# google-deepmind/spriteworld

Measured on AMD Instinct MI355X. Metric: env-steps/sec (incl. 64x64 RGB render) at 8192 envs, higher is better.
Workload: dtype i32 fixed-point raster/resample + f64 state

## Files before the change

include/swb.h:

```cpp
#ifndef SWB_H_
#define SWB_H_

#include <stdint.h>

#ifdef __cplusplus
extern "C" {
#endif

#define SWB_MAX_SPRITES 64
#define SWB_MAX_TASKS 8
#define SWB_MAX_SHAPES 32
#define SWB_MAX_SHAPE_VERTS 64
#define SWB_MAX_CUTS 4
#define SWB_MAX_CELLS ((SWB_MAX_CUTS + 1) * (SWB_MAX_CUTS + 1))

enum swb_status {
  SWB_OK = 0,
  SWB_ERR_INVALID = -1,
  SWB_ERR_HIP = -2,
  SWB_ERR_NO_DEVICE = -3,
  SWB_ERR_STATE = -4
};

enum swb_action_space {
// ... 261 lines not shown

#define SWB_ALL_STEPS (-1)
int swb_rollout_step_frames(swb_handle h, int32_t M, int32_t step, const int32_t* cand_dev, uint8_t* obs_dev, uint8_t* error_dev,
                            void* stream);

#define SWB_CONTAINED_MAX_TRIES 1024
enum swb_action_sampling { SWB_SAMPLE_UNIFORM = 0, SWB_SAMPLE_ON_SPRITE = 1 };
typedef struct swb_sampled_actions {
  void* actions;
  double* position;
  int32_t* sprite;
  int32_t* tries;
} swb_sampled_actions;
int swb_sample_actions(swb_handle h, int32_t mode, uint64_t seed, uint64_t first_env, const swb_sampled_actions* out, void* stream);

typedef struct swb_rollout_sampled_outputs {
  void*    actions;
  int32_t* sprite;
  int32_t* tries;
} swb_rollout_sampled_outputs;
int swb_rollout_sampled(swb_handle h, int32_t mode , uint64_t seed, uint64_t first_env,
                        int32_t M, int32_t K, int32_t keep_steps, const swb_rollout_outputs* out,
                        const swb_rollout_step_outputs* steps, const swb_rollout_sampled_outputs* sampled, void* stream);

int swb_trim_run_lists(swb_handle h, int32_t* run_cap_out, void* stream);

int swb_list_stats(swb_handle h, int64_t* kept, int64_t* built, void* stream);

int swb_frame_stats(swb_handle h, int64_t* copied, int64_t* filled, int64_t* resampled, void* stream);
int swb_frame_cycles(swb_handle h, int64_t* out3, void* stream);

int swb_split_stats(swb_handle h, int64_t* whole, int64_t* bands, int64_t* whole_copies, void* stream);

int swb_factors(swb_handle h, double* factors_dev, void* stream);

int swb_get_env_state(swb_handle h, int32_t env, int32_t* out5, void* stream);
int swb_get_sprite_types(swb_handle h, int32_t env, int32_t sprite, int32_t* flags, void* stream);

int swb_get_state(swb_handle h, const swb_state* host_state, void* stream);
int swb_set_positions(swb_handle h, const double* x_host, const double* y_host, void* stream);

typedef struct swb_snapshot {
  double *x, *y;
  int32_t *n_sprites, *pool_entry, *step_count, *episode, *pool_base, *pool_len;
  uint8_t *reset_next;
} swb_snapshot;
enum swb_state_source { SWB_STATE_LIVE = 0, SWB_STATE_ROLLOUT_END = 1 };
int swb_pool_id(swb_handle h, uint64_t* id);
int swb_save_state(swb_handle h, int32_t source, const int32_t* index_dev, int32_t C, const swb_snapshot* snap, void* stream);
int swb_load_state(swb_handle h, const swb_snapshot* snap, int32_t C, const int32_t* slot_dev, uint64_t pool_id,
                   int32_t* rejected_dev, void* stream);

int swb_copy_pool(swb_handle dst, swb_handle src, const int32_t* pool_base_host, const int32_t* pool_len_host, void* stream);

enum swb_sprite_attr { SWB_ATTR_SHAPE = 0, SWB_ATTR_ANGLE = 1, SWB_ATTR_SCALE = 2 };
int swb_set_sprite_attr(swb_handle h, int32_t env, int32_t sprite, int32_t attr, double value, const double* delta,
                        const int8_t* label, void* stream);

int swb_set_sprite_cell_labels(swb_handle h, int32_t env, int32_t sprite, const int8_t* cells, void* stream);

int swb_get_sprite(swb_handle h, int32_t env, int32_t sprite, int32_t* shape, double* angle, double* scale, int32_t* n_verts,
                   double* path_xy, void* stream);

int swb_sprite_path_op(int32_t attr, double a, double b, int32_t n, const double* in_xy, double* out_xy);

typedef struct swb_variant_info {
  int32_t nw;
  int32_t ncol;
  int32_t vs;
  int32_t lds_bytes_per_wave;
  int32_t waves_per_simd;
  int32_t resample_waves_per_simd;
  int32_t n_bands;
  int32_t n_column_groups;
  int32_t run_cap;
  int32_t paint_in_cover;
  int32_t arena_units;
  int32_t large_frames;
  int32_t many_sprites;
  int32_t reserved_;
  int64_t run_list_bytes;
  int64_t frame_cache_bytes;
  int32_t split_bands;
  int32_t split_pad_;
} swb_variant_info;
int swb_variant(swb_handle h, swb_variant_info* out);
const char* swb_build_id(void);

int swb_timing_enable(swb_handle h, int32_t enable);
int swb_step_time_ms(swb_handle h, double* total_ms, int64_t* launches);
int swb_kernel_times_ms(swb_handle h, double* cover_ms, double* resample_ms, int64_t* launches);

#ifdef __cplusplus
}
#endif
#endif
```

spriteworld_amd/_abi.py:

```python
import ctypes as C

SWB_MAX_SPRITES = 64
SWB_TUNED_SPRITES = 16
SWB_MAX_TASKS = 8
SWB_MAX_SHAPES = 32
SWB_MAX_SHAPE_VERTS = 64
SWB_MAX_GROUPS = 8
SWB_MAX_CUTS = 4
SWB_MAX_CELLS = (SWB_MAX_CUTS + 1) * (SWB_MAX_CUTS + 1)
SWB_MAX_CANDIDATES = 12

ACTION_SELECT_MOVE, ACTION_DRAG_AND_DROP, ACTION_EMBODIED = 0, 1, 2
TASK_NO_REWARD, TASK_FIND_GOAL, TASK_CLUSTERING = 0, 1, 2
AGG_SUM, AGG_MAX, AGG_MIN, AGG_MEAN = 0, 1, 2, 3
TERM_ALL, TERM_ANY = 0, 1
STEP_FIRST, STEP_MID, STEP_LAST = 0, 1, 2
ENV_ERR_DB_ZERO, ENV_ERR_DB_LABELS, ENV_ERR_SPAN_OVERFLOW = 1, 2, 4
ATTR_SHAPE, ATTR_ANGLE, ATTR_SCALE = 0, 1, 2
SAMPLE_UNIFORM, SAMPLE_ON_SPRITE = 0, 1
SWB_CONTAINED_MAX_TRIES = 1024


class SwbTask(C.Structure):
  _fields_ = [
# ... 117 lines not shown
      ('x', C.c_void_p),
      ('y', C.c_void_p),
      ('n_sprites', C.c_void_p),
      ('pool_entry', C.c_void_p),
      ('step_count', C.c_void_p),
      ('reset_next', C.c_void_p),
      ('episode', C.c_void_p),
  ]


class SwbSnapshot(C.Structure):
  _fields_ = [
      ('x', C.c_void_p),
      ('y', C.c_void_p),
      ('n_sprites', C.c_void_p),
      ('pool_entry', C.c_void_p),
      ('step_count', C.c_void_p),
      ('episode', C.c_void_p),
      ('pool_base', C.c_void_p),
      ('pool_len', C.c_void_p),
      ('reset_next', C.c_void_p),
  ]


STATE_LIVE, STATE_ROLLOUT_END = 0, 1


class SwbVariantInfo(C.Structure):
  _fields_ = [('nw', C.c_int32), ('ncol', C.c_int32), ('vs', C.c_int32), ('lds_bytes_per_wave', C.c_int32),
              ('waves_per_simd', C.c_int32), ('resample_waves_per_simd', C.c_int32), ('n_bands', C.c_int32),
              ('n_column_groups', C.c_int32), ('run_cap', C.c_int32), ('paint_in_cover', C.c_int32),
              ('arena_units', C.c_int32), ('large_frames', C.c_int32), ('many_sprites', C.c_int32), ('reserved_', C.c_int32),
              ('run_list_bytes', C.c_int64), ('frame_cache_bytes', C.c_int64),
              ('split_bands', C.c_int32), ('split_pad_', C.c_int32)]


FACTOR_UNIFORM_F32, FACTOR_UNIFORM_INT, FACTOR_DISCRETE = 0, 1, 2


class SwbFactor(C.Structure):
  _fields_ = [
      ('kind', C.c_int32),
      ('n', C.c_int32),
      ('lo', C.c_double),
      ('hi', C.c_double),
      ('cand', C.c_double * SWB_MAX_CANDIDATES),
  ]


FACTOR_ORDER = ('x', 'y', 'scale', 'angle', 'c0', 'c1', 'c2', 'x_vel', 'y_vel')
SWB_N_FACTORS = len(FACTOR_ORDER)
SWB_MAX_HOLDOUTS = 2


class SwbHoldout(C.Structure):
  _fields_ = [
      ('redraw_mask', C.c_uint32),
      ('box_mask', C.c_uint32),
      ('lo', C.c_double * SWB_N_FACTORS),
      ('hi', C.c_double * SWB_N_FACTORS),
  ]


class SwbSpriteGroup(C.Structure):

  def factor(self, key):
    return self.factors[FACTOR_ORDER.index(key)]
# ... 203 lines not shown
```

spriteworld_amd/csrc/swb.hip:

```cpp
#include <hip/hip_runtime.h>

#include <algorithm>
#include <atomic>
#include <cmath>
#include <cstdarg>
#include <cstdio>
#include <cstdlib>
#include <cstring>
#include <memory>
#include <string>
#include <vector>

#include "swb_kernels.hip.inc"
#include "swb_pow.hip.inc"
#include "swb_sampler.hip.inc"

extern template __global__ void swb_cover_kernel<20, false>(const swb_params);
extern template __global__ void swb_cover_kernel<20, true>(const swb_params);

namespace {

thread_local std::string g_err;

int fail(int code, const char* fmt, ...) {
// ... 890 lines not shown
    if (per_xcd >= 2 && (per_xcd & (per_xcd - 1)) == 0 && rs_waves <= (long long)h->cus * 4 * SWB_RS_WAVES_PER_SIMD && !getenv("SWB_NO_SNAKE"))
      while ((1 << p.deal_shift) < per_xcd) ++p.deal_shift;
    if (const char* x = getenv("SWB_DEAL_SHIFT")) p.deal_shift = std::max(0, atoi(x));
  }
  h->run_cap_worst = std::max(4, p.S + 1) * p.Hc + 1;
  p.run_cap = h->run_cap_worst;
  if (const char* x = getenv("SWB_RUN_CAP")) p.run_cap = std::max(8, atoi(x));
  if (const char* x = getenv("SWB_ARENA_UNITS")) h->arena_override = std::max(0, atoi(x));
  const size_t NS = (size_t)p.N * p.S;
  if (h->d_x.fill(nullptr, NS) || h->d_y.fill(nullptr, NS) || h->d_nspr.fill(nullptr, p.N) || h->d_entry.fill(nullptr, p.N) ||
      h->d_step_count.fill(nullptr, p.N) || h->d_episode.fill(nullptr, p.N) || h->d_reset_next.fill(nullptr, p.N))
    return SWB_ERR_HIP;
  if (getenv("SWB_LIST_STATS")) {
    if (h->d_list_stats.fill(nullptr, 2) || h->d_frame_stats.fill(nullptr, 6)) return SWB_ERR_HIP;
    p.list_stats = h->d_list_stats;
    p.frame_stats = h->d_frame_stats;
    if (h->split_bands) {
      if (h->d_split_stats.fill(nullptr, 3)) return SWB_ERR_HIP;
      p.split_stats = h->d_split_stats;
    }
  }
  h->copy_cost = h->split_bands ? SWB_SPLIT_COPY_COST : SWB_COPY_COST;
  if (const char* x = getenv("SWB_COPY_COST")) h->copy_cost = std::max(0, atoi(x));
  if (p.AA != 1 && !h->large_frames && !h->no_keep_lists && !getenv("SWB_NO_FRAME_CACHE")) {
    const size_t bytes = (size_t)p.N * p.Wo * p.Ho * 3;
    if (hipMalloc(reinterpret_cast<void**>(&h->d_frame_cache.ptr), bytes) == hipSuccess) {
      h->d_frame_cache.count = bytes;
      p.frame_cache = h->d_frame_cache;
    } else {
      h->d_frame_cache.ptr = nullptr;
      (void)hipGetLastError();
    }
  }
  p.max_spans = SWB_MIN_SPANS;
  if (const char* ms = getenv("SWB_MAX_SPANS")) p.max_spans = atoi(ms) < SWB_MIN_SPANS ? SWB_MIN_SPANS : atoi(ms);
  p.span_cap = p.max_spans;
  if (const char* sc = getenv("SWB_LDS_SPAN_CAP")) p.span_cap = std::max(0, std::min(atoi(sc), p.max_spans));
  p.ovf_cap = std::min(p.Wc / 2 + 1, 32);
  p.ovf = nullptr;
  p.x = h->d_x; p.y = h->d_y; p.nspr = h->d_nspr; p.entry = h->d_entry; p.step_count = h->d_step_count;
  p.episode = h->d_episode; p.reset_next = h->d_reset_next;
  *out = owner.release();
  return SWB_OK;
}

int swb_destroy(swb_handle h) {
  if (!h) return SWB_OK;
  (void)hipSetDevice(h->device);
  for (auto* list : {&h->events, &h->event_pool})
    for (auto& ev : *list) { (void)hipEventDestroy(ev.e0); (void)hipEventDestroy(ev.e1); (void)hipEventDestroy(ev.e2); }
  delete h;
  return SWB_OK;
}

int swb_upload_shapes(swb_handle h, const double* verts, const int32_t* offsets, int32_t n_shapes) {
  if (!h || !verts || !offsets) return fail(SWB_ERR_INVALID, "null argument");
  bump_list_epoch(h);
  if (n_shapes < 1 || n_shapes > SWB_MAX_SHAPES) return fail(SWB_ERR_INVALID, "n_shapes must be in [1, %d]", SWB_MAX_SHAPES);
  HIP_TRY(hipSetDevice(h->device));
  int maxv = 0;
  for (int i = 0; i < n_shapes; ++i) {
    const int n = offsets[i + 1] - offsets[i];
    if (n < 3 || n > SWB_MAX_SHAPE_VERTS) return fail(SWB_ERR_INVALID, "shape %d has %d vertices (3..%d supported)", i, n, SWB_MAX_SHAPE_VERTS);
    if (n > maxv) maxv = n;
  }
  std::vector<double> dmin(n_shapes, 0.0);
// ... 1149 lines not shown
  if (shape) *shape = r.shape[sprite];
  if (angle) *angle = r.angle[sprite];
  if (scale) *scale = r.scale[sprite];
  if (n_verts) *n_verts = nv;
  if (path_xy) memcpy(path_xy, r.cpath.data() + (size_t)sprite * SWB_MAX_SHAPE_VERTS * 2, (size_t)nv * 16);
  return SWB_OK;
}

int swb_variant(swb_handle h, swb_variant_info* out) {
  if (!h || !out) return fail(SWB_ERR_INVALID, "null argument");
  if (h->large_frames) {
    const variant* v0 = &kVariants[0];
    out->nw = v0->nw; out->ncol = 1; out->vs = 0;
    out->lds_bytes_per_wave = (int32_t)lds_per_wave(h, v0, nullptr);
    out->waves_per_simd = SWB_COVER_WAVES(v0->nw);
    out->resample_waves_per_simd = 0;
    out->n_bands = 0;
    out->n_column_groups = 0;
    out->run_cap = 0;
    out->paint_in_cover = 0;
    out->arena_units = 0;
    out->large_frames = 1;
    out->many_sprites = h->many_sprites ? 1 : 0;
    out->reserved_ = 0;
    if (h->many_sprites) {
      out->nw = 0;
      out->lds_bytes_per_wave = (int32_t)sizeof(swb_ms_lds);
      out->waves_per_simd = 0;
    }
    out->run_list_bytes = 0;
    out->frame_cache_bytes = 0;
    out->split_bands = 0;
    out->split_pad_ = 0;
    return SWB_OK;
  }
  const variant* v = pick_variant(h->p.Wc);
  if (!v) return fail(SWB_ERR_INVALID, "canvas %dx%d not supported", h->p.Wc, h->p.Hc);
  int vs = 0;
  (void)pick_resample(h->p.AA, h->vslots, &vs);
  out->nw = v->nw; out->ncol = 1; out->vs = vs;
  out->lds_bytes_per_wave = (int32_t)lds_per_wave(h, v, nullptr);
  out->waves_per_simd = SWB_COVER_WAVES(v->nw);
  out->resample_waves_per_simd = SWB_RS_WAVES_PER_SIMD;
  out->n_bands = h->split_bands ? 1 : (h->p.nbands ? h->p.nbands : h->nbands);
  out->split_bands = h->split_bands ? (h->p.nbands ? h->p.nbands : h->nbands) : 0;
  out->split_pad_ = 0;
  out->n_column_groups = h->p.ncg;
  out->run_cap = h->p.run_cap;
  out->paint_in_cover = paints_in_cover(h, v) ? 1 : 0;
  out->arena_units = h->d_runs ? h->p.arena_units : 0;
  out->large_frames = 0;
  out->many_sprites = 0;
  out->reserved_ = 0;
  out->run_list_bytes = h->d_runs ? ((int64_t)h->p.arena_base + h->p.arena_units + 4) * 8 : 0;
  out->frame_cache_bytes = (int64_t)h->d_frame_cache.count;
  return SWB_OK;
}

#ifndef SWB_BUILD_ID
#define SWB_BUILD_ID "unknown"
#endif
const char* swb_build_id(void) { return SWB_BUILD_ID; }

int swb_timing_enable(swb_handle h, int32_t enable) {
  if (!h) return fail(SWB_ERR_INVALID, "null handle");
  HIP_TRY(hipSetDevice(h->device));
  if (flush_timing(h)) return SWB_ERR_HIP;
  h->timing = enable != 0;
  h->timed_ms = 0.0;
  h->timed_cover_ms = 0.0;
  h->timed_launches = 0;
  return SWB_OK;
}

int swb_step_time_ms(swb_handle h, double* total_ms, int64_t* launches) {
  if (!h) return fail(SWB_ERR_INVALID, "null handle");
  HIP_TRY(hipSetDevice(h->device));
  if (flush_timing(h)) return SWB_ERR_HIP;
  if (total_ms) *total_ms = h->timed_ms;
// ... 16 lines not shown
```

spriteworld_amd/csrc/swb_kernels.hip.inc:

```
#include <hip/hip_runtime.h>
#include <stdint.h>

#include "../../include/swb.h"

#define SWB_WAVE 64
#ifndef SWB_WORD_GROUPS
#define SWB_WORD_GROUPS 4
#endif
#ifndef SWB_AES_MIN_ITERS
#define SWB_AES_MIN_ITERS 4
#endif
#ifndef SWB_AES_MAX_NARROW_NW
#define SWB_AES_MAX_NARROW_NW 10
#endif
#ifndef SWB_COVER_WAVES_PER_SIMD
#define SWB_COVER_WAVES_PER_SIMD 5
#endif
#ifndef SWB_COVER_WAVES_PER_SIMD_NARROW
#define SWB_COVER_WAVES_PER_SIMD_NARROW 6
#endif
#ifndef SWB_COVER_WAVES_PER_SIMD_WIDE
#define SWB_COVER_WAVES_PER_SIMD_WIDE 4
#endif
#ifndef SWB_RS_WAVES_PER_SIMD
// ... 69 lines not shown
  const uint32_t* v_break;
  const int32_t* cg_lo;
  const int32_t* cg_hi;
  uint32_t* cost_cnt;
  int32_t* cost_list;
  int32_t cost_cap;
  int32_t cost_range0;
  int32_t parity;
  int32_t deal_shift;
  int32_t* ccost_list;
  int32_t cover_order;
  int32_t cphase;
  int32_t prio_div;
  int32_t prio_levels;
  int32_t paint_in_cover;
  int32_t band_tasks;
  uint8_t* ov_flag;
  const int32_t* ov_shape;
  const double* ov_scale;
  const double* ov_angle;
  const int8_t* ov_label;
  const double* ov_cpath;
  const int8_t* ov_cell_label;
  uint32_t list_epoch;
  uint32_t list_pad_;
  unsigned long long* list_stats;
  uint8_t* frame_cache;
  unsigned long long* frame_stats;
  int32_t obs_aligned16;
  int32_t copy_cost;
  int32_t split_bands;
  int32_t split_when;
  int32_t split_carry;
  int32_t split_pad_;
  unsigned long long* split_stats;
};

template <typename T>
using cptr = const T __attribute__((address_space(4)))*;
template <typename T>
__device__ __forceinline__ cptr<T> as_const(const T* q) { return (cptr<T>)(uintptr_t)q; }

__device__ __forceinline__ int lane_id() { return threadIdx.x & (SWB_WAVE - 1); }
__device__ __forceinline__ int rfl(int v) { return __builtin_amdgcn_readfirstlane(v); }
__device__ __forceinline__ float rflf(float v) { return __int_as_float(__builtin_amdgcn_readfirstlane(__float_as_int(v))); }
__device__ __forceinline__ double rfld(double v) {
  const long long b = __double_as_longlong(v);
  const int lo = __builtin_amdgcn_readfirstlane((int)(b & 0xffffffffll));
  const int hi = __builtin_amdgcn_readfirstlane((int)(b >> 32));
  return __longlong_as_double(((long long)hi << 32) | (unsigned int)lo);
}
__device__ __forceinline__ double readlane_d(double v, int src) {
  const long long b = __double_as_longlong(v);
  const int lo = __builtin_amdgcn_readlane((int)(b & 0xffffffffll), src);
  const int hi = __builtin_amdgcn_readlane((int)(b >> 32), src);
  return __longlong_as_double(((long long)hi << 32) | (unsigned int)lo);
}
__device__ __forceinline__ void wave_sync() {
  __builtin_amdgcn_fence(__ATOMIC_ACQ_REL, "wavefront");
  __builtin_amdgcn_wave_barrier();
}
__device__ __forceinline__ int wave_min_i(int v) {
  for (int o = 32; o > 0; o >>= 1) v = min(v, __shfl_xor(v, o, 64));
  return v;
}
__device__ __forceinline__ int wave_max_i(int v) {
  for (int o = 32; o > 0; o >>= 1) v = max(v, __shfl_xor(v, o, 64));
// ... 1364 lines not shown
        }                                                                                                         \
      } while (0)
      SWB_LIST_SPAN(rs.s0, 0 < cnt);
      SWB_LIST_SPAN(rs.s1, 1 < cnt);
      SWB_LIST_SPAN(rs.s2, 2 < cnt);
      for (int i = SWB_REG_SPANS; i < maxc; ++i) SWB_LIST_SPAN(lane_span(p, spans, ovf, rs, i, l), i < cnt);
#undef SWB_LIST_SPAN
      if (start && fc > SWB_REG_SPANS && ((fc - 3) & 1)) dst[2 * (2 + ((fc - 3) >> 1)) + 1] = 0u;
    }
    while (next_band_g < p.nbands) {
      const int y0 = as_const(p.band_y0)[next_band_g];
      if (y0 > yb + 63) break;
      const int at = base_g + ((y0 <= yb || !room) ? 0 : __builtin_amdgcn_readlane(excl, (y0 - yb) & 63));
      if (l == 0) hdr[SWB_RHDR_GROUPS + g * SWB_RHDR_GSTRIDE + 1 + next_band_g] = (uint32_t)at;
      if (bst && l == 0) bst[g * SWB_BST_STRIDE + next_band_g] = (uint32_t)at;
      ++next_band_g;
    }
    const int cost_g = SWB_RUN_COST * __popcll(__ballot(start)) + SWB_UNIT_COST * (total - __popcll(__ballot(contin)));
    if (l == g) { base_l = room ? base_g + total : base_g; band_l = (int)((meta_g & ~15u) | (uint32_t)next_band_g); cost_l += room ? cost_g : 0; }
  }
}

#define SWB_RESCAN_WITH_OVERFLOW_SLOT()                                                          \
  if (__ballot((err & SWB_INT_NEED_SLOT) != 0u)) {                                               \
    err &= ~SWB_INT_NEED_SLOT;                                                                   \
    if (rfl(*ovf) == -1) {                                                                       \
      if (l == 0) *ovf = ovf_slot_alloc(p);                                                      \
      wave_sync();                                                                               \
      if (rfl(*ovf) >= 0) { yb -= 64; continue; }                                                \
    }                                                                                            \
    err |= SWB_ENV_ERR_SPAN_OVERFLOW;                                                            \
  }

template <int NW, bool OV = false, bool PAINT = false>
__global__ void __launch_bounds__(SWB_WAVE, SWB_COVER_WAVES(NW))
swb_cover_kernel(const swb_params p) {
  static_assert(!PAINT || NW == 2, "painting in the cover kernel: images of up to 64 columns at anti_aliasing = 1");
  extern __shared__ __attribute__((aligned(16))) unsigned char smem[];
  const int l = lane_id();
  const uint32_t cycles0 = (uint32_t)__builtin_amdgcn_s_memtime();
  int env = blockIdx.x;
  uint32_t predicted = 0u, prio_q = 0u;
  int prio = 0;
  const int ph = p.cphase, ph_prev = ph == 0 ? 2 : ph - 1, ph_next = ph == 2 ? 0 : ph + 1;
  uint32_t filing_words_l = 0u;
  if (p.cost_cnt != nullptr && l < ((!PAINT && p.split_bands) ? 4 : 3))
    filing_words_l = p.cost_cnt[l == 0 ? SWB_COST_WORD_KEY_LO(p.parity) : (l == 1 ? SWB_COST_WORD_KEY_SCALE(p.parity) : ((PAINT || l == 2) ? SWB_COST_WORD_COVER_SHIFT(ph) : SWB_COST_WORD_SPLIT(p.parity)))];
  if (p.ccost_list) cover_cost_housekeeping(p, ph_prev, ph, ph_next);
  if (p.arena_head != nullptr && blockIdx.x == 0 && l == 0) p.arena_head[p.parity ^ 1] = 0u;
  if (p.cover_order) {
    const int sh = (int)(blockIdx.x & (SWB_COST_SHARDS - 1)), cap = (p.N + SWB_COST_SHARDS - 1) / SWB_COST_SHARDS;
    int bucket = 0;
    env = cost_ordered_entry(p.cost_cnt + cost_row1(ph_prev, sh),
                             as_const(p.ccost_list) + (size_t)(ph_prev * SWB_COST_SHARDS + sh) * SWB_COST_BUCKETS * cap, cap,
                             (int)(blockIdx.x >> 3), &bucket);
    if (env < 0) return;
    prio_q = (p.prio_levels & 2) ? as_const(p.cost_cnt)[SWB_COST_WORD_COVER_PRIO(ph)] : 0u;
    if (prio_q) predicted = (uint32_t)(2 * bucket + 1) << (as_const(p.cost_cnt)[SWB_COST_WORD_COVER_SHIFT(ph_prev)] - 1u);
  }
  auto file_cover_cost = [&]() __attribute__((always_inline)) {
    if (p.ccost_list) {
      const uint32_t cycles = (uint32_t)__builtin_amdgcn_s_memtime() - cycles0;
      const uint32_t width = (uint32_t)__builtin_amdgcn_readlane((int)filing_words_l, 2);
      if (l == 0) {
        const int key = (int)min(cycles >> width, (uint32_t)(SWB_COST_BUCKETS - 1));
        const int sh = env & (SWB_COST_SHARDS - 1);
// ... 59 lines not shown
    if (k < vtotal) {
      double cx, cy;
      bool from_table = true;
      if constexpr (OV) {
        if (es.ov) {
          const double* q = p.ov_cpath + (((size_t)env * S + sid) * SWB_MAX_SHAPE_VERTS + i) * 2;
          cx = q[0]; cy = q[1];
          from_table = false;
        }
      }
      if (from_table) centered_vertex(p, so, i, sc, ca, sa, cx, cy);
      cpath[k] = make_double2(cx, cy);
    }
  }
  wave_sync();
  SWB_HOOK_PHASE_END(3)

  auto hit = [&](int s2, double tx, double ty) __attribute__((always_inline)) {
    return contains_point_wave(cpath + __builtin_amdgcn_readlane(voff_l, s2), __builtin_amdgcn_readlane(nv_l, s2), tx, ty);
  };
  const step_cost sc = act_and_move(p, env, es, hit);
  const double px = es.px, py = es.py;
  SWB_HOOK_PHASE_END(4)
  if (p.render_only != 1) {
    err |= finish_step<OV>(p, env, es, sc, tscratch);
    wave_sync();
  }
  SWB_HOOK_PHASE_END(5)
  if (p.obs == nullptr) {
    if (l == 0 && p.error && err) p.error[env] |= (uint8_t)err;
    return;
  }

  [[maybe_unused]] auto file_lists = [&](int cost_l, const uint32_t* bst, uint32_t built_cycles, bool copies) __attribute__((always_inline)) {
    const bool whole = p.split_bands && (copies || __builtin_amdgcn_readlane((int)filing_words_l, 3) == 0);
    const bool bt = bst != nullptr && !whole;
    const int ntask = bt ? p.ncg * p.nbands : p.ncg;
    const bool file0 = p.cost_cnt != nullptr && l < ntask, file1 = p.ccost_list != nullptr && l == 0;
    const int sh = env & (SWB_COST_SHARDS - 1);
    int task_cost = cost_l, task_bits = l << 24;
    if (bt) {
      wave_sync();
      const int g2 = min(l / p.nbands, p.ncg - 1), b2 = l - (l / p.nbands) * p.nbands;
      const uint32_t* bg = bst + g2 * SWB_BST_STRIDE;
      const int u0 = (int)bg[b2], u1 = (int)bg[min(b2 + 1, p.nbands)], u2 = (int)bg[min(b2 + 2, p.nbands)];
      task_cost = 4 * max((u1 - u0) + (p.AA == 1 ? 0 : (((u2 - u1) * 5) >> 4)), 0);
      task_bits = (g2 << 24) | (b2 << 26);
    }
    if (whole) task_bits |= SWB_TASK_WHOLE;
    if (copies) task_cost = p.copy_cost;
    const int key0 = cost_key(task_cost, (uint32_t)__builtin_amdgcn_readlane((int)filing_words_l, 0), (uint32_t)__builtin_amdgcn_readlane((int)filing_words_l, 1));
    int key1 = 0;
    uint32_t cycles = built_cycles;
    if (p.ccost_list) {
      if (built_cycles == 0u) cycles = (uint32_t)__builtin_amdgcn_s_memtime() - cycles0;
      const uint32_t width = (uint32_t)__builtin_amdgcn_readlane((int)filing_words_l, 2);
      key1 = (int)min(cycles >> width, (uint32_t)(SWB_COST_BUCKETS - 1));
      if (l == 0 && (cycles >> width) >= (uint32_t)SWB_COST_BUCKETS) atomicMax(&p.cost_cnt[SWB_COST_WORD_COVER_MAX(ph, sh)], cycles);
    }
    uint32_t pos0 = 0u, pos1 = 0u;
    if (copies) { if (file0 && l == 0) pos0 = atomicAdd(&p.cost_cnt[cost_row0(p.parity, sh) + key0], (uint32_t)ntask); }
    else if (file0) pos0 = atomicAdd(&p.cost_cnt[cost_row0(p.parity, sh) + key0], 1u);
    if (file1) pos1 = atomicAdd(&p.cost_cnt[cost_row1(ph, sh) + key1], 1u);
    if (p.split_bands && !copies && p.cost_cnt != nullptr && l == 0) atomicAdd(&p.cost_cnt[SWB_COST_WORD_SPLIT_CNT(p.parity, sh, (env >> 3) & (SWB_COST_BUCKETS - 1))], (uint32_t)p.ncg);
    if (copies) pos0 = (uint32_t)__builtin_amdgcn_readlane((int)pos0, 0) + (uint32_t)l;
    if (file0) p.cost_list[((size_t)(p.parity * SWB_COST_SHARDS + sh) * SWB_COST_BUCKETS + key0) * p.cost_cap + pos0] = env | task_bits;
    if (file1) p.ccost_list[((size_t)(ph * SWB_COST_SHARDS + sh) * SWB_COST_BUCKETS + key1) * ((p.N + SWB_COST_SHARDS - 1) / SWB_COST_SHARDS) + pos1] = env;
    if (l == 0) ovf_slot_release(p, ovf);
    if (p.error) {
      uint32_t e = err & ~SWB_INT_NEED_SLOT;
      for (int o = 32; o > 0; o >>= 1) e |= (uint32_t)__shfl_xor((int)e, o, 64);
      if (l == 0 && e) p.error[env] |= (uint8_t)e;
    }
    return cycles;
  };

  if constexpr (!PAINT) {
    bool keep = false;
    uint32_t keep_words_l = 0u;
    if (p.list_epoch != 0u) {
      if (l <= SWB_MAX_CG + 2) keep_words_l = L->outrow[l];
      keep = (uint32_t)__builtin_amdgcn_readlane((int)keep_words_l, SWB_MAX_CG) == p.list_epoch && __ballot(es.first) == 0ull && !sc.changed;
    }
    if (p.list_stats != nullptr && l == 0) atomicAdd(&p.list_stats[keep ? 0 : 1], 1ull);
    if (keep) {
      const uint32_t frame_word_was = (uint32_t)__builtin_amdgcn_readlane((int)keep_words_l, SWB_MAX_CG + 2);
      const uint32_t frame_word = p.frame_cache ? min(frame_word_was + 1u, 2u) : 0u;
      uint32_t* bst = nullptr;
      const bool files_whole = p.split_bands && (frame_word == 2u || __builtin_amdgcn_readlane((int)filing_words_l, 3) == 0);
      if (p.band_tasks && !files_whole) {
        bst = L->outrow + 64;
        const uint32_t* hg = p.rhdr + (size_t)env * SWB_RHDR_DWORDS + SWB_RHDR_GROUPS;
        const int g = l / SWB_BST_STRIDE, b = l - g * SWB_BST_STRIDE;
        if (g < p.ncg && b <= p.nbands) bst[l] = hg[g * SWB_RHDR_GSTRIDE + (b < p.nbands ? 1 + b : 0)];
      }
      if (l == 0 && frame_word != frame_word_was) p.rhdr[(size_t)env * SWB_RHDR_DWORDS + SWB_RHDR_FRAME] = frame_word;
      file_lists((int)keep_words_l, bst, max((uint32_t)__builtin_amdgcn_readlane((int)keep_words_l, SWB_MAX_CG + 1), 1u), frame_word == 2u);
      return;
    }
  }

  build_all_edges<NW>(p, L, edges, cpath, spans, n, vtotal, voff_l, nv_l, px, py, dmin_l, scale_l, rgb_reg, err);
#pragma unroll
  for (int w = 0; w < SWB_NWA(NW); ++w) { L->T[w][l] = 0u; L->Px[w][l] = 0u; }
  wave_sync();

  if (n >= SWB_EAGER_OVF_SPRITES && l == 0) *ovf = ovf_slot_alloc(p);
  int sp_ymin = 0x7fffffff, sp_ymax = -0x7fffffff, sp_e0 = 0;
  uint32_t sp_a = 0u;
  if (l < n) {
    const sprite_rec r = L->spr[l];
    static_assert(SWB_TUNED_SPRITES * SWB_MAX_SHAPE_VERTS <= 4096 && SWB_MAX_SHAPE_VERTS <= 64, "packing of sp_e0 / lanes per edge");
    const int lanes_per_edge = max(64 / max(r.n_edges, 2), 1);
    sp_ymin = r.ymin; sp_ymax = r.ymax;
    sp_e0 = r.edge_off | (((65536 + lanes_per_edge - 1) / lanes_per_edge) << 12);
    sp_a = (uint32_t)r.w0 | ((uint32_t)r.w1 << 5) | ((uint32_t)r.n_edges << 10) | ((uint32_t)min(r.max_edge_rows, 127) << 17) |
           ((uint32_t)lanes_per_edge << 24);
  }
  uint32_t* hdr = p.rhdr + (size_t)env * SWB_RHDR_DWORDS;
  if (l < SWB_TUNED_SPRITES && !PAINT) {
    hdr[l] = (uint32_t)(((int)(rgb_reg & 255) - (int)(p.bg & 255)) & 0x3ff) |
             ((uint32_t)(((int)((rgb_reg >> 8) & 255) - (int)((p.bg >> 8) & 255)) & 0x3ff) << 10) |
             ((uint32_t)(((int)((rgb_reg >> 16) & 255) - (int)((p.bg >> 16) & 255)) & 0x3ff) << 20);
    hdr[SWB_TUNED_SPRITES + l] = rgb_reg;
  }
  SWB_HOOK_PHASE_END(1)
  reprioritise();

  if constexpr (PAINT) {
    const int nd1 = (p.Wo * 3) >> 2;
// ... 60 lines not shown
  uint32_t* runs_env = p.runs + (size_t)env * p.ncg * p.run_cap * 2;
  int base_l = 0, band_l = 0, cost_l = 0;
  static_assert(64 + SWB_MAX_CG * SWB_BST_STRIDE <= 132, "the band starts borrow wave_lds::outrow behind the scatter's 64 slots");
  uint32_t* const bst = p.band_tasks ? L->outrow + 64 : nullptr;
  const bool skip_empty = (p.bg == 0u) || p.AA == 1;
  for (int yb = 0;; yb += 64) {
    if (skip_empty) {
      int v = (l < n && sp_ymax >= yb) ? max(sp_ymin, yb) : 0x7fffffff;
      v = min(v, __builtin_amdgcn_update_dpp(0x7fffffff, v, 0x111, 0xf, 0xf, false));
      v = min(v, __builtin_amdgcn_update_dpp(0x7fffffff, v, 0x112, 0xf, 0xf, false));
      v = min(v, __builtin_amdgcn_update_dpp(0x7fffffff, v, 0x114, 0xf, 0xf, false));
      v = min(v, __builtin_amdgcn_update_dpp(0x7fffffff, v, 0x118, 0xf, 0xf, false));
      yb = __builtin_amdgcn_readlane(v, SWB_TUNED_SPRITES - 1);
    }
    if (yb >= p.Hc) break;
    row_spans rs;
    coverage_batch2<NW>(p, L, edges, spans, ovf, n, yb, sp_ymin, sp_ymax, sp_a, sp_e0, rs, err);
    SWB_RESCAN_WITH_OVERFLOW_SLOT()
    emit_runs(p, spans, ovf, rs, yb, env, runs_env, hdr, bst, base_l, band_l, cost_l, err);
    reprioritise();
  }
  if (l < p.ncg) {
    hdr[SWB_RHDR_GROUPS + l * SWB_RHDR_GSTRIDE] = (uint32_t)base_l;
    for (int b = band_l & 15; b < p.nbands; ++b) hdr[SWB_RHDR_GROUPS + l * SWB_RHDR_GSTRIDE + 1 + b] = (uint32_t)base_l;
    if (bst) for (int b = band_l & 15; b <= p.nbands; ++b) bst[l * SWB_BST_STRIDE + b] = (uint32_t)base_l;
    *reinterpret_cast<uint2*>(runs_env + (size_t)l * p.run_cap * 2 + 2 * (long long)base_l) = make_uint2(0xffffu, 0u);
  }
  {
    const bool flawed_l = (err & ~SWB_INT_NEED_SLOT) != 0u || (l < p.ncg && ((uint32_t)band_l >> 4) != 0u);
    const bool stamped = p.list_epoch != 0u && __ballot(flawed_l) == 0ull;
    if (l <= SWB_MAX_CG) hdr[SWB_RHDR_COST + l] = l < SWB_MAX_CG ? (uint32_t)cost_l : (stamped ? p.list_epoch : 0u);
    if (l == SWB_MAX_CG + 2) hdr[SWB_RHDR_FRAME] = 0u;
  }
  const uint32_t own_cycles = file_lists(cost_l, bst, 0u, false);
  if (l == 0 && p.list_epoch != 0u) hdr[SWB_RHDR_CYCLES] = own_cycles;
  }
}

template <typename T, int BATCH>
__device__ __forceinline__ void copy_frame_rect_as(const unsigned char* src, unsigned char* dst, uint32_t row_bytes, uint32_t seg_bytes, int rows) {
  const int l = lane_id();
  const int cpr = (int)(seg_bytes / (uint32_t)sizeof(T)), total = rows * cpr;
  const int step_rows = 64 / cpr, step_cols = 64 - step_rows * cpr;
  int row = l / cpr, col = l - row * cpr;
  for (int base = 0; base < total; base += 64 * BATCH) {
    T v[BATCH];
    uint32_t off[BATCH];
#pragma unroll
    for (int j = 0; j < BATCH; ++j) {
      off[j] = (uint32_t)row * row_bytes + (uint32_t)col * (uint32_t)sizeof(T);
      if (base + 64 * j + l < total) v[j] = *reinterpret_cast<const T*>(src + off[j]);
      row += step_rows; col += step_cols;
      if (col >= cpr) { col -= cpr; ++row; }
    }
#pragma unroll
    for (int j = 0; j < BATCH; ++j)
      if (base + 64 * j + l < total) *reinterpret_cast<T*>(dst + off[j]) = v[j];
  }
}
typedef uint32_t swb_c16 __attribute__((ext_vector_type(4)));
__device__ __forceinline__ void copy_frame_rect(const unsigned char* src, unsigned char* dst, uint32_t row_bytes, uint32_t seg_bytes, int rows, bool aligned16) {
  if (aligned16) copy_frame_rect_as<swb_c16, 6>(src, dst, row_bytes, seg_bytes, rows);
  else copy_frame_rect_as<uint32_t, 8>(src, dst, row_bytes, seg_bytes, rows);
}
typedef uint32_t swb_u4 __attribute__((ext_vector_type(4), aligned(8)));
typedef int32_t swb_i8 __attribute__((ext_vector_type(8), aligned(32)));
template <int VS>
__global__ void __launch_bounds__(SWB_WAVE* SWB_RS_WAVES_PER_BLOCK, SWB_RS_WAVES_PER_SIMD)
swb_resample_kernel(const swb_params p) {
  extern __shared__ __attribute__((aligned(16))) unsigned char smem[];
  const int wave = rfl(threadIdx.x >> 6);
  const int l = lane_id();
  const int task = blockIdx.x * SWB_RS_WAVES_PER_BLOCK + wave;
  int band = blockIdx.y;
  int env = task < p.N ? task : -1, g = blockIdx.z;
  bool whole = false;
  if (p.cost_cnt) {
    const int first = dealt_block(p, (int)(blockIdx.x >> 3), (int)(gridDim.x >> 3)) * SWB_RS_WAVES_PER_BLOCK;
    int filed = 0;
    env = cost_ordered_env(p, p.parity, (int)(blockIdx.x & (SWB_COST_SHARDS - 1)), first + wave, &filed);
    if (env >= 0) {
      whole = (env & SWB_TASK_WHOLE) != 0;
      if (p.band_tasks) band = rfl((env >> 26) & 7);
      g = (env >> 24) & 3; env &= 0xffffff;
    }
    if (blockIdx.y == 0) cost_housekeeping(p, (int)blockIdx.x, wave);
    if (p.split_bands && first >= filed) return;
  }
  int32_t* pfx = reinterpret_cast<int32_t*>(smem);
  for (int i = threadIdx.x; i < p.h_pfx_len; i += blockDim.x) pfx[i] = p.h_pfx[i];
  __syncthreads();
  if (env < 0) return;
  const int o_lo = as_const(p.band_lo)[band], o_hi = as_const(p.band_lo)[whole ? p.nbands : band + 1];
  if (o_lo >= o_hi) return;
  cptr<uint32_t> hdr = as_const(p.rhdr) + (size_t)env * SWB_RHDR_DWORDS;
  const uint32_t frame_mode = p.frame_cache ? hdr[SWB_RHDR_FRAME] : 0u;
  const uint32_t rect_row_bytes = 3u * (uint32_t)p.Wo, rect_seg_bytes = 3u * (uint32_t)min(64, p.Wo - 64 * g);
  const size_t frame_off = (size_t)env * p.Wo * p.Ho * 3 + (size_t)(p.Ho - o_hi) * rect_row_bytes + 192u * (uint32_t)g;
  const uint32_t cycles0 = p.frame_stats ? (uint32_t)__builtin_amdgcn_s_memtime() : 0u;
  if (p.frame_stats && l == 0 && (!p.split_bands || whole || band == 0)) atomicAdd(&p.frame_stats[frame_mode == 2u ? 0 : (frame_mode == 1u ? 1 : 2)], 1ull);
  if (p.split_stats && l == 0) atomicAdd(&p.split_stats[!whole ? 1 : (frame_mode == 2u ? 2 : 0)], 1ull);
  if (frame_mode == 2u) {
    copy_frame_rect(p.frame_cache + frame_off, p.obs + frame_off, rect_row_bytes, rect_seg_bytes, o_hi - o_lo, p.obs_aligned16 != 0);
    if (p.frame_stats && l == 0) atomicAdd(&p.frame_stats[3], (unsigned long long)((uint32_t)__builtin_amdgcn_s_memtime() - cycles0));
    return;
  }
  const uint32_t dpk_reg = (l < SWB_TUNED_SPRITES) ? p.rhdr[(size_t)env * SWB_RHDR_DWORDS + l] : 0u;
  uint32_t uo = 8u * hdr[SWB_RHDR_GROUPS + g * SWB_RHDR_GSTRIDE + 1 + band];
  const uint32_t u_end = 8u * hdr[SWB_RHDR_GROUPS + g * SWB_RHDR_GSTRIDE + ((!whole && band + 1 < p.nbands) ? 2 + band : 0)];
  const uint32_t prio_shift = p.cost_cnt ? as_const(p.cost_cnt)[SWB_COST_WORD_PRIO_SHIFT(p.parity)] : 0u;
  int prio = prio_shift ? (int)min((u_end - uo) >> prio_shift, 3u) : 0;
  if (p.frame_stats && l == 0) atomicAdd(&p.frame_stats[5], (unsigned long long)(u_end - uo));
  if (prio == 3) __builtin_amdgcn_s_setprio(3);
  else if (prio == 2) __builtin_amdgcn_s_setprio(2);
  else if (prio == 1) __builtin_amdgcn_s_setprio(1);
  cptr<unsigned char> runs = reinterpret_cast<cptr<unsigned char>>(as_const(p.runs) + ((size_t)env * p.ncg + g) * p.run_cap * 2);
  cptr<unsigned char> vpfx = reinterpret_cast<cptr<unsigned char>>(as_const(p.v_pfx));
  const int bg0 = p.bg & 255, bg1 = (p.bg >> 8) & 255, bg2 = (p.bg >> 16) & 255;
  const int o = min(64 * g + l, p.Wo - 1);
  const int hxmin = p.h_xmin[o], hcnt = p.h_cnt[o], htbl = p.h_tbl[o];
// ... 767 lines not shown
```

Baseline: 78.88 million.

## Copy cached frames inside cover kernel instead of filing resample tasks

When an env's frame is unchanged and cached, the cover kernel now copies the whole cached frame to the observation buffer itself and skips filing resample tasks for it. Resample blocks with no filed work exit early when cover copies are enabled. This moves copy work from the resample launch into cover, which is meant to cut task-queue overhead and idle resample waves. It is enabled by default only when env count is large relative to cover slots, and it may lengthen the cover kernel.

```diff
diff --git a/include/swb.h b/include/swb.h
--- a/include/swb.h
+++ b/include/swb.h
@@ -317,6 +317,7 @@
 
 int swb_split_stats(swb_handle h, int64_t* whole, int64_t* bands, int64_t* whole_copies, void* stream);
 
+
 int swb_factors(swb_handle h, double* factors_dev, void* stream);
 
 int swb_get_env_state(swb_handle h, int32_t env, int32_t* out5, void* stream);
@@ -368,6 +369,8 @@
   int64_t frame_cache_bytes;
   int32_t split_bands;
   int32_t split_pad_;
+  int32_t cover_copies;
+  int32_t cover_pad_;
 } swb_variant_info;
 int swb_variant(swb_handle h, swb_variant_info* out);
 const char* swb_build_id(void);
diff --git a/spriteworld_amd/_abi.py b/spriteworld_amd/_abi.py
--- a/spriteworld_amd/_abi.py
+++ b/spriteworld_amd/_abi.py
@@ -173,7 +173,8 @@
               ('n_column_groups', C.c_int32), ('run_cap', C.c_int32), ('paint_in_cover', C.c_int32),
               ('arena_units', C.c_int32), ('large_frames', C.c_int32), ('many_sprites', C.c_int32), ('reserved_', C.c_int32),
               ('run_list_bytes', C.c_int64), ('frame_cache_bytes', C.c_int64),
-              ('split_bands', C.c_int32), ('split_pad_', C.c_int32)]
+              ('split_bands', C.c_int32), ('split_pad_', C.c_int32),
+              ('cover_copies', C.c_int32), ('cover_pad_', C.c_int32)]
 
 
 FACTOR_UNIFORM_F32, FACTOR_UNIFORM_INT, FACTOR_DISCRETE = 0, 1, 2
diff --git a/spriteworld_amd/csrc/swb.hip b/spriteworld_amd/csrc/swb.hip
--- a/spriteworld_amd/csrc/swb.hip
+++ b/spriteworld_amd/csrc/swb.hip
@@ -946,6 +946,13 @@
       (void)hipGetLastError();
     }
   }
+  {
+    const variant* v = h->large_frames ? nullptr : pick_variant(p.Wc);
+    const long long slots = (long long)cus * 4 * (v ? SWB_COVER_WAVES(v->nw) : 1);
+    const bool can = p.frame_cache && p.cost_cnt && v;
+    p.cover_copies = (can && p.N > 4 * slots) ? 1 : 0;
+    if (const char* x = getenv("SWB_COVER_COPY")) p.cover_copies = (can && atoi(x) != 0) ? 1 : 0;
+  }
   p.max_spans = SWB_MIN_SPANS;
   if (const char* ms = getenv("SWB_MAX_SPANS")) p.max_spans = atoi(ms) < SWB_MIN_SPANS ? SWB_MIN_SPANS : atoi(ms);
   p.span_cap = p.max_spans;
@@ -2161,6 +2168,8 @@
     out->frame_cache_bytes = 0;
     out->split_bands = 0;
     out->split_pad_ = 0;
+    out->cover_copies = 0;
+    out->cover_pad_ = 0;
     return SWB_OK;
   }
   const variant* v = pick_variant(h->p.Wc);
@@ -2174,6 +2183,8 @@
   out->n_bands = h->split_bands ? 1 : (h->p.nbands ? h->p.nbands : h->nbands);
   out->split_bands = h->split_bands ? (h->p.nbands ? h->p.nbands : h->nbands) : 0;
   out->split_pad_ = 0;
+  out->cover_copies = h->p.cover_copies;
+  out->cover_pad_ = 0;
   out->n_column_groups = h->p.ncg;
   out->run_cap = h->p.run_cap;
   out->paint_in_cover = paints_in_cover(h, v) ? 1 : 0;
diff --git a/spriteworld_amd/csrc/swb_kernels.hip.inc b/spriteworld_amd/csrc/swb_kernels.hip.inc
--- a/spriteworld_amd/csrc/swb_kernels.hip.inc
+++ b/spriteworld_amd/csrc/swb_kernels.hip.inc
@@ -125,7 +125,7 @@
   int32_t split_bands;
   int32_t split_when;
   int32_t split_carry;
-  int32_t split_pad_;
+  int32_t cover_copies;
   unsigned long long* split_stats;
 };
 
@@ -1556,6 +1556,34 @@
     err |= SWB_ENV_ERR_SPAN_OVERFLOW;                                                            \
   }
 
+template <typename T, int BATCH>
+__device__ __forceinline__ void copy_frame_rect_as(const unsigned char* src, unsigned char* dst, uint32_t row_bytes, uint32_t seg_bytes, int rows) {
+  const int l = lane_id();
+  const int cpr = (int)(seg_bytes / (uint32_t)sizeof(T)), total = rows * cpr;
+  const int step_rows = 64 / cpr, step_cols = 64 - step_rows * cpr;
+  int row = l / cpr, col = l - row * cpr;
+  for (int base = 0; base < total; base += 64 * BATCH) {
+    T v[BATCH];
+    uint32_t off[BATCH];
+#pragma unroll
+    for (int j = 0; j < BATCH; ++j) {
+      off[j] = (uint32_t)row * row_bytes + (uint32_t)col * (uint32_t)sizeof(T);
+      if (base + 64 * j + l < total) v[j] = *reinterpret_cast<const T*>(src + off[j]);
+      row += step_rows; col += step_cols;
+      if (col >= cpr) { col -= cpr; ++row; }
+    }
+#pragma unroll
+    for (int j = 0; j < BATCH; ++j)
+      if (base + 64 * j + l < total) *reinterpret_cast<T*>(dst + off[j]) = v[j];
+  }
+}
+typedef uint32_t swb_c16 __attribute__((ext_vector_type(4)));
+template <int BATCH16 = 6, int BATCH4 = 8>
+__device__ __forceinline__ void copy_frame_rect(const unsigned char* src, unsigned char* dst, uint32_t row_bytes, uint32_t seg_bytes, int rows, bool aligned16) {
+  if (aligned16) copy_frame_rect_as<swb_c16, BATCH16>(src, dst, row_bytes, seg_bytes, rows);
+  else copy_frame_rect_as<uint32_t, BATCH4>(src, dst, row_bytes, seg_bytes, rows);
+}
+
 template <int NW, bool OV = false, bool PAINT = false>
 __global__ void __launch_bounds__(SWB_WAVE, SWB_COVER_WAVES(NW))
 swb_cover_kernel(const swb_params p) {
@@ -1681,11 +1709,11 @@
     return;
   }
 
-  [[maybe_unused]] auto file_lists = [&](int cost_l, const uint32_t* bst, uint32_t built_cycles, bool copies) __attribute__((always_inline)) {
+  [[maybe_unused]] auto file_lists = [&](int cost_l, const uint32_t* bst, uint32_t built_cycles, bool copies, bool copied) __attribute__((always_inline)) {
     const bool whole = p.split_bands && (copies || __builtin_amdgcn_readlane((int)filing_words_l, 3) == 0);
     const bool bt = bst != nullptr && !whole;
     const int ntask = bt ? p.ncg * p.nbands : p.ncg;
-    const bool file0 = p.cost_cnt != nullptr && l < ntask, file1 = p.ccost_list != nullptr && l == 0;
+    const bool file0 = p.cost_cnt != nullptr && l < ntask && !copied, file1 = p.ccost_list != nullptr && l == 0;
     const int sh = env & (SWB_COST_SHARDS - 1);
     int task_cost = cost_l, task_bits = l << 24;
     if (bt) {
@@ -1736,15 +1764,29 @@
       const uint32_t frame_word_was = (uint32_t)__builtin_amdgcn_readlane((int)keep_words_l, SWB_MAX_CG + 2);
       const uint32_t frame_word = p.frame_cache ? min(frame_word_was + 1u, 2u) : 0u;
       uint32_t* bst = nullptr;
+      const bool cover_copy = p.cover_copies != 0 && frame_word == 2u;
+      if (cover_copy) {
+        const uint32_t copy0 = p.frame_stats ? (uint32_t)__builtin_amdgcn_s_memtime() : 0u;
+        const uint32_t frame_bytes = 3u * (uint32_t)p.Wo * (uint32_t)p.Ho;
+        const size_t frame_off = (size_t)env * frame_bytes;
+        copy_frame_rect<4, 4>(p.frame_cache + frame_off, p.obs + frame_off, frame_bytes, frame_bytes, 1, p.obs_aligned16 != 0);
+        if (l == 0) {
+          if (p.frame_stats) {
+            atomicAdd(&p.frame_stats[0], (unsigned long long)(p.split_bands ? p.ncg : p.ncg * p.nbands));
+            atomicAdd(&p.frame_stats[3], (unsigned long long)((uint32_t)__builtin_amdgcn_s_memtime() - copy0));
+          }
+          if (p.split_stats) atomicAdd(&p.split_stats[2], (unsigned long long)p.ncg);
+        }
+      }
       const bool files_whole = p.split_bands && (frame_word == 2u || __builtin_amdgcn_readlane((int)filing_words_l, 3) == 0);
-      if (p.band_tasks && !files_whole) {
+      if (p.band_tasks && !files_whole && !cover_copy) {
         bst = L->outrow + 64;
         const uint32_t* hg = p.rhdr + (size_t)env * SWB_RHDR_DWORDS + SWB_RHDR_GROUPS;
         const int g = l / SWB_BST_STRIDE, b = l - g * SWB_BST_STRIDE;
         if (g < p.ncg && b <= p.nbands) bst[l] = hg[g * SWB_RHDR_GSTRIDE + (b < p.nbands ? 1 + b : 0)];
       }
       if (l == 0 && frame_word != frame_word_was) p.rhdr[(size_t)env * SWB_RHDR_DWORDS + SWB_RHDR_FRAME] = frame_word;
-      file_lists((int)keep_words_l, bst, max((uint32_t)__builtin_amdgcn_readlane((int)keep_words_l, SWB_MAX_CG + 1), 1u), frame_word == 2u);
+      file_lists((int)keep_words_l, bst, max((uint32_t)__builtin_amdgcn_readlane((int)keep_words_l, SWB_MAX_CG + 1), 1u), frame_word == 2u, cover_copy);
       return;
     }
   }
@@ -1871,37 +1913,11 @@
     if (l <= SWB_MAX_CG) hdr[SWB_RHDR_COST + l] = l < SWB_MAX_CG ? (uint32_t)cost_l : (stamped ? p.list_epoch : 0u);
     if (l == SWB_MAX_CG + 2) hdr[SWB_RHDR_FRAME] = 0u;
   }
-  const uint32_t own_cycles = file_lists(cost_l, bst, 0u, false);
+  const uint32_t own_cycles = file_lists(cost_l, bst, 0u, false, false);
   if (l == 0 && p.list_epoch != 0u) hdr[SWB_RHDR_CYCLES] = own_cycles;
   }
 }
 
-template <typename T, int BATCH>
-__device__ __forceinline__ void copy_frame_rect_as(const unsigned char* src, unsigned char* dst, uint32_t row_bytes, uint32_t seg_bytes, int rows) {
-  const int l = lane_id();
-  const int cpr = (int)(seg_bytes / (uint32_t)sizeof(T)), total = rows * cpr;
-  const int step_rows = 64 / cpr, step_cols = 64 - step_rows * cpr;
-  int row = l / cpr, col = l - row * cpr;
-  for (int base = 0; base < total; base += 64 * BATCH) {
-    T v[BATCH];
-    uint32_t off[BATCH];
-#pragma unroll
-    for (int j = 0; j < BATCH; ++j) {
-      off[j] = (uint32_t)row * row_bytes + (uint32_t)col * (uint32_t)sizeof(T);
-      if (base + 64 * j + l < total) v[j] = *reinterpret_cast<const T*>(src + off[j]);
-      row += step_rows; col += step_cols;
-      if (col >= cpr) { col -= cpr; ++row; }
-    }
-#pragma unroll
-    for (int j = 0; j < BATCH; ++j)
-      if (base + 64 * j + l < total) *reinterpret_cast<T*>(dst + off[j]) = v[j];
-  }
-}
-typedef uint32_t swb_c16 __attribute__((ext_vector_type(4)));
-__device__ __forceinline__ void copy_frame_rect(const unsigned char* src, unsigned char* dst, uint32_t row_bytes, uint32_t seg_bytes, int rows, bool aligned16) {
-  if (aligned16) copy_frame_rect_as<swb_c16, 6>(src, dst, row_bytes, seg_bytes, rows);
-  else copy_frame_rect_as<uint32_t, 8>(src, dst, row_bytes, seg_bytes, rows);
-}
 typedef uint32_t swb_u4 __attribute__((ext_vector_type(4), aligned(8)));
 typedef int32_t swb_i8 __attribute__((ext_vector_type(8), aligned(32)));
 template <int VS>
@@ -1924,7 +1940,7 @@
       g = (env >> 24) & 3; env &= 0xffffff;
     }
     if (blockIdx.y == 0) cost_housekeeping(p, (int)blockIdx.x, wave);
-    if (p.split_bands && first >= filed) return;
+    if ((p.split_bands | p.cover_copies) && first >= filed) return;
   }
   int32_t* pfx = reinterpret_cast<int32_t*>(smem);
   for (int i = threadIdx.x; i < p.h_pfx_len; i += blockDim.x) pfx[i] = p.h_pfx[i];
```

Result: no change. 78.53 million (-0.4%).
